# KenHBS/LDA_thesis

Measured on AMD Instinct MI355X. Metric: million tokens resampled/sec (Gibbs sweep), higher is better.
Workload: dtype f64-exact (fp32 tier 0 + fp64 tiers: the drawn topic is the fp64 pipeline's)

## Files before the change

### lda_thesis_amd/csrc/build_info.hpp

```cpp
#pragma once
#ifdef LLDA_MARGIN0
#define LLDA_INFO_MARGIN0 LLDA_BUILD_MARGIN0
#else
#define LLDA_INFO_MARGIN0 0
#endif
#ifdef LLDA_WAVES
#define LLDA_INFO_WAVES LLDA_BUILD_WAVES
#else
#define LLDA_INFO_WAVES 0
#endif
#ifdef LLDA_MARGIN0_WIDE
#define LLDA_INFO_MARGIN0_WIDE LLDA_BUILD_MARGIN0_WIDE
#else
#define LLDA_INFO_MARGIN0_WIDE 0
#endif
#ifdef ABL_NOLOAD
#define LLDA_INFO_NOLOAD LLDA_BUILD_ABL_NOLOAD
#else
#define LLDA_INFO_NOLOAD 0
#endif
#ifdef ABL_NOCOMMIT
#define LLDA_INFO_NOCOMMIT LLDA_BUILD_ABL_NOCOMMIT
#else
#define LLDA_INFO_NOCOMMIT 0
#endif
#ifdef ABL_WIDE_NOROW
#define LLDA_INFO_WIDE_NOROW LLDA_BUILD_ABL_WIDE_NOROW
#else
#define LLDA_INFO_WIDE_NOROW 0
#endif
#ifdef ABL_WIDE_NOADDLOAD
#define LLDA_INFO_WIDE_NOADDLOAD LLDA_BUILD_ABL_WIDE_NOADDLOAD
#else
#define LLDA_INFO_WIDE_NOADDLOAD 0
#endif
#ifdef ABL_NOFMA
#define LLDA_INFO_NOFMA LLDA_BUILD_ABL_NOFMA
#else
#define LLDA_INFO_NOFMA 0
#endif
#ifdef ABL_EXTRA_LDS_BYTES
#define LLDA_INFO_EXTRA_LDS LLDA_BUILD_ABL_EXTRA_LDS
#else
#define LLDA_INFO_EXTRA_LDS 0
#endif
#ifdef QUAD_PROFILE
#define LLDA_INFO_QUAD_PROFILE LLDA_BUILD_QUAD_PROFILE
#else
#define LLDA_INFO_QUAD_PROFILE 0
#endif
#ifdef LLDA_BUDGET_MARKS
#define LLDA_INFO_BUDGET_MARKS LLDA_BUILD_BUDGET_MARKS
#else
#define LLDA_INFO_BUDGET_MARKS 0
#endif
#ifdef LLDA_QUAD_PRIO
#define LLDA_INFO_QUAD_PRIO LLDA_BUILD_QUAD_PRIO
#else
#define LLDA_INFO_QUAD_PRIO 0
#endif
#define LLDA_BUILD_INFO_BITS (LLDA_INFO_QUAD_PRIO | LLDA_INFO_QUAD_PROFILE | LLDA_INFO_BUDGET_MARKS | LLDA_INFO_MARGIN0 | LLDA_INFO_WAVES | LLDA_INFO_MARGIN0_WIDE | LLDA_INFO_NOLOAD | LLDA_INFO_NOCOMMIT | \
                              LLDA_INFO_WIDE_NOROW | LLDA_INFO_WIDE_NOADDLOAD | LLDA_INFO_NOFMA | LLDA_INFO_EXTRA_LDS)
```

### lda_thesis_amd/csrc/kernel_quad.hpp

```cpp
#pragma once

namespace {

constexpr float LLDA_MARGIN0_QUAD = 0x1.ap-18f;
constexpr float QM_L = 1.05f * 32.0f * 0x1p-24f, QM_T = 1.05f * 39.0f * 0x1p-24f, QM_P = 1.05f * 37.0f * 0x1p-24f, QM_TOT = 1.05f * 0.25f * 0x1p-24f;
#define QLDS(arr, rho, t) (arr)[(rho) >> 2][t][(rho) & 3]
constexpr int QT = 32;
#ifdef LLDA_QUAD_PRIO
constexpr int QP_TOP = (LLDA_QUAD_PRIO) / 100 % 10, QP_DEC = (LLDA_QUAD_PRIO) / 10 % 10, QP_BULK = (LLDA_QUAD_PRIO) % 10;
#else
constexpr int QP_TOP = 3, QP_DEC = 0, QP_BULK = 2;
#endif
constexpr int QNT = 128;

template <int LB>
struct QuadGeo {
    static constexpr int LPD = 1 << LB;
    static constexpr int G = 2 * LPD;
    static constexpr int KP = 32 * LPD;
    static constexpr int IS = 3 + LB;
    static constexpr int DPW = 64 / LPD;
    static constexpr uint64_t GM = LPD == 64 ? ~0ull : ((1ull << LPD) - 1);
    static constexpr uint32_t KEY_NONE = 0xFC000u | 31u << 9 | (uint32_t)(KP - 1);
};

template <int LB>
__device__ __forceinline__ int quad_rho(int pos) { return ((pos >> LB) & 0x18) | ((pos & 3) << 1) | ((pos >> 2) & 1); }
constexpr int quad_rho_of(int i, int e, int c) { return 8 * i + 2 * c + e; }

template <int LB>
__device__ __forceinline__ uint32_t quad_min_key(uint32_t key)
{
    if constexpr (LB == 4)
        asm volatile("s_nop 1\n\tv_min_u32_dpp %0, %0, %0 row_ror:8 row_mask:0xf bank_mask:0xf\n\ts_nop 1\n\t"
                     "v_min_u32_dpp %0, %0, %0 row_ror:4 row_mask:0xf bank_mask:0xf\n\ts_nop 1\n\t"
                     "v_min_u32_dpp %0, %0, %0 row_ror:2 row_mask:0xf bank_mask:0xf\n\ts_nop 1\n\t"
                     "v_min_u32_dpp %0, %0, %0 row_ror:1 row_mask:0xf bank_mask:0xf" : "+v"(key));
    else if constexpr (LB == 3)
        asm volatile("s_nop 1\n\tv_min_u32_dpp %0, %0, %0 row_half_mirror row_mask:0xf bank_mask:0xf\n\ts_nop 1\n\t"
                     "v_min_u32_dpp %0, %0, %0 quad_perm:[1,0,3,2] row_mask:0xf bank_mask:0xf\n\ts_nop 1\n\t"
                     "v_min_u32_dpp %0, %0, %0 quad_perm:[2,3,0,1] row_mask:0xf bank_mask:0xf" : "+v"(key));
    else
        asm volatile("s_nop 1\n\tv_min_u32_dpp %0, %0, %0 quad_perm:[1,0,3,2] row_mask:0xf bank_mask:0xf\n\ts_nop 1\n\t"
                     "v_min_u32_dpp %0, %0, %0 quad_perm:[2,3,0,1] row_mask:0xf bank_mask:0xf" : "+v"(key));
    return key;
}

template <int LB>
struct QuadCounts {
    const int (*s_ndk)[QNT][4];
    const int *s_nk0;
    int t;
    int e;
    int g;
    bool st;
    __device__ __forceinline__ int word(int s) const { return QLDS(s_ndk, 8 * (s >> 2) + 2 * (s & 3) + e, t); }
    __device__ __forceinline__ int nd(int s) const { return word(s) & 0xffff; }
    __device__ __forceinline__ int nk(int s) const
    {
        const int w = word(s);
        return s_nk0[pos_of<QuadGeo<LB>::G, 16>(g, s)] + (w & 0xffff) - (int)((uint32_t)w >> 16);
    }
    __device__ __forceinline__ bool stats() const { return st; }
    __device__ __forceinline__ bool count_unsure() const { return false; }
};

template <int LB, bool PAD>
__device__ __noinline__ int quad_cold(const int (*s_ndk)[QNT][4], const int *s_nk0, int tbase, int w, int f, int zo, uint32_t ra,
                                      uint32_t rb, int lane, int64_t d, const KParams *P)
{
    constexpr int G = QuadGeo<LB>::G;
    const int g = lane & (G - 1);
    int x[16];
    gload_lane_row<G, 16>(P->n_kw, (int64_t)w * QuadGeo<LB>::KP, g, x);
    int lo, so;
    lane_slot_of<G, 16>(zo, lo, so);
#pragma unroll
    for (int s = 0; s < 16; ++s) x[s] -= (g == lo && s == so) ? f : 0;
    const QuadCounts<LB> dc{s_ndk, s_nk0, tbase + (g >> 1), g & 1, g, lane < G};
    if constexpr (PAD) return cold_tiers_acc<G, 16, true, false>(dc, x, P->lab_mask[d * G + g], uniform53(ra, rb), g, lane, P);
    else return cold_tiers_acc<G, 16, false, true>(dc, x, 0xFFFFu, uniform53(ra, rb), g, lane, P);
}

typedef float q_v2f __attribute__((ext_vector_type(2)));
typedef float q_v32f __attribute__((ext_vector_type(32)));

template <int LB, bool PAD = false>
__device__ __forceinline__ uint64_t quad_draw(const q_v32f &xv, const q_v2f (&pa)[16], float u, float margin_rel, float margin_data, float beta,
                                              int lq, int &zn)
{
    const q_v2f b2 = {beta, beta};
    q_v2f Q[16];
    LLDA_MARK("scores");
#pragma unroll
    for (int a = 0; a < 16; ++a) {
        const q_v2f x2 = {xv[2 * a], xv[2 * a + 1]};
        const q_v2f nb = x2 + b2;
        if (a == 0) Q[0] = nb * pa[0];
        else Q[a] = __builtin_elementwise_fma(nb, pa[a], Q[a - 1]);
    }
    LLDA_MARK("lane_scan");
    __builtin_amdgcn_s_setprio(QP_DEC);
    const float X0 = Q[15].x + Q[15].y;
    float X = X0;
    float tot = X0, prev;
    if constexpr (LB == 4) {
        X += dpp_f32<DPP_ROW_SHR + 1>(X);
        X += dpp_f32<DPP_ROW_SHR + 2>(X);
        X += dpp_f32<DPP_ROW_SHR + 4>(X);
        X += dpp_f32<DPP_ROW_SHR + 8>(X);
        tot += dpp_f32<DPP_ROW_ROR + 8>(tot);
        tot += dpp_f32<DPP_ROW_ROR + 4>(tot);
        tot += dpp_f32<DPP_ROW_ROR + 2>(tot);
        tot += dpp_f32<DPP_ROW_ROR + 1>(tot);
        prev = __int_as_float(__builtin_amdgcn_update_dpp(0, __float_as_int(X), DPP_ROW_SHR + 1, 0xF, 0xF, true));
    } else {
        const float m1 = lq >= 1 ? 1.0f : 0.0f, m2 = lq >= 2 ? 1.0f : 0.0f;
        X = __builtin_fmaf(dpp_f32<DPP_ROW_SHR + 1>(X), m1, X);
        X = __builtin_fmaf(dpp_f32<DPP_ROW_SHR + 2>(X), m2, X);
        if constexpr (LB == 3) {
            const float m4 = lq >= 4 ? 1.0f : 0.0f;
            X = __builtin_fmaf(dpp_f32<DPP_ROW_SHR + 4>(X), m4, X);
            tot += dpp_f32<DPP_HALF_MIRROR>(tot);
        }
        tot += dpp_f32<DPP_XOR1>(tot);
        tot += dpp_f32<DPP_XOR2>(tot);
        prev = dpp_f32<DPP_ROW_SHR + 1>(X) * m1;
    }
    LLDA_MARK("threshold");
    const float t = u * tot;
    const float tg = t - prev;
    const float md = __builtin_fmaf(QM_L, X0, __builtin_fmaf(QM_T, t, __builtin_fmaf(QM_P, prev, QM_TOT * tot)));
    const float margin = __builtin_fmaf(tot, margin_rel, margin_data * md);
    const float lo0 = tg - margin, hi0 = tg + margin;
    LLDA_MARK("search");
    const bool c0 = Q[15].x <= lo0;
    const float dA = c0 ? Q[15].x : 0.0f;
    const float lo = lo0 - dA, hi = hi0 - dA;
    float q[16];
#pragma unroll
    for (int a = 0; a < 16; ++a) q[a] = c0 ? Q[a].y : Q[a].x;
    const bool c5 = q[15] <= lo;
    float ub = c5 ? __int_as_float(0x7f800000) : q[15];
    const bool c1 = q[7] <= lo;
    ub = c1 ? ub : q[7];
    const float m2 = c1 ? q[11] : q[3];
    const float a1 = c1 ? q[9] : q[1], a5 = c1 ? q[13] : q[5];
    const float e0 = c1 ? q[8] : q[0], e2 = c1 ? q[10] : q[2], e4 = c1 ? q[12] : q[4], e6 = c1 ? q[14] : q[6];
    const bool c2 = m2 <= lo;
    ub = c2 ? ub : m2;
    const float m3 = c2 ? a5 : a1;
    const float g0 = c2 ? e4 : e0, g2 = c2 ? e6 : e2;
    const bool c3 = m3 <= lo;
    ub = c3 ? ub : m3;
    const float m4 = c3 ? g2 : g0;
    const bool c4 = m4 <= lo;
    ub = c4 ? ub : m4;
    uint64_t bad_total;
    asm("v_cmp_class_f32_e64 %0, %1, %2" : "=s"(bad_total) : "v"(tot - margin), "v"(0x2FF));
    uint64_t unsure = __ballot(!(ub > hi)) | bad_total;
    LLDA_MARK("pick");
    constexpr uint32_t I1 = 2u << QuadGeo<LB>::IS, I0 = 1u << QuadGeo<LB>::IS;
    const uint32_t p = (c1 ? (I1 | 16u << 9) : 0u) | (c2 ? (I0 | 8u << 9) : 0u) | (c3 ? (2u | 4u << 9) : 0u) | (c4 ? (1u | 2u << 9) : 0u) |
                       (c0 ? (4u | 1u << 9) : 0u) | ((uint32_t)lq << 3) | ((uint32_t)lq << 14);
    uint32_t key = c5 ? QuadGeo<LB>::KEY_NONE : p;
    key = quad_min_key<LB>(key);
    zn = (int)(key & 0x3FFFu);
    if constexpr (PAD) unsure |= __ballot(key == QuadGeo<LB>::KEY_NONE);
    return unsure;
}

template <int LB, bool PAD = false>
__device__ __forceinline__ uint64_t quad_tier1(const q_v32f &xv, const int (*s_ndk)[QNT][4], const int *s_nk0, int tid, int lq, double u,
                                               double alpha, double beta, double vbeta, double margin_rel, uint32_t vm, int &zn)
{
    double W[QT];
    double run = 0.0;
#pragma unroll
    for (int k = 0; k < QT; ++k) {
        const int e = k >> 4, a = k & 15, i = a >> 2, c = a & 3;
        const int rho = quad_rho_of(i, e, c);
        const int w = QLDS(s_ndk, rho, tid);
        const int nd = w & 0xffff, nk = s_nk0[(i << QuadGeo<LB>::IS) | (lq << 3) | (e << 2) | c] + nd - (int)((uint32_t)w >> 16);
        const double den = (double)nk + vbeta;
        double y = (double)__builtin_amdgcn_rcpf((float)den);
        y = __builtin_fma(__builtin_fma(-den, y, 1.0), y, y);
        y = __builtin_fma(__builtin_fma(-den, y, 1.0), y, y);
        const double ws = ((double)nd + alpha) * (((double)xv[rho] + beta) * y);
        run = run + (((vm >> k) & 1u) ? ws : 0.0);
        W[k] = run;
    }
    constexpr int LPD = QuadGeo<LB>::LPD;
    const double X = group_scan<LPD>(run, lq);
    const double tot = bcast_last<LPD>(X, tid & 63);
    double prev = dpp_f64<DPP_ROW_SHR + 1>(X);
    if constexpr (LB < 4) prev = lq ? prev : 0.0;
    const double tg = u * tot - prev;
    const double margin = tot * margin_rel;
    const double lo = tg - margin, hi = tg + margin;
    int cnt_lo = 0, cnt_hi = 0;
#pragma unroll
    for (int k = 0; k < QT; ++k) {
        cnt_lo += (W[k] <= lo) ? 1 : 0;
        cnt_hi += (W[k] <= hi) ? 1 : 0;
    }
    uint64_t unsure = __ballot((cnt_lo != cnt_hi) || !(tot > 0.0) || !(margin < tot));
    const uint32_t k = (uint32_t)cnt_lo;
    const uint32_t i_ = (k >> 2) & 3u, e_ = (k >> 4) & 1u, c_ = k & 3u;
    const uint32_t p = (i_ << QuadGeo<LB>::IS) | ((uint32_t)lq << 3) | (e_ << 2) | c_ | ((8u * i_ + 2u * c_ + e_) << 9) | ((uint32_t)lq << 14);
    uint32_t key = cnt_lo >= QT ? QuadGeo<LB>::KEY_NONE : p;
    key = quad_min_key<LB>(key);
    zn = (int)(key & 0x3FFFu);
    if constexpr (PAD) unsure |= __ballot(key == QuadGeo<LB>::KEY_NONE);
    return unsure;
}

struct QuadSite { int v, f, zo, c, zn, lo, so, w; };

#ifdef QUAD_PROFILE
#define QP_DECL uint32_t qp_t = 0, qp_acc[8] = {0, 0, 0, 0, 0, 0, 0, 0}
#define QP_START() do { __builtin_amdgcn_sched_barrier(0); qp_t = (uint32_t)__builtin_amdgcn_s_memtime(); __builtin_amdgcn_sched_barrier(0); } while (0)
#define QP_MARK(k) do { __builtin_amdgcn_sched_barrier(0); const uint32_t qp_n = (uint32_t)__builtin_amdgcn_s_memtime(); \
                        qp_acc[k] += qp_n - qp_t; qp_t = qp_n; __builtin_amdgcn_sched_barrier(0); } while (0)
#else
#define QP_DECL
#define QP_START()
#define QP_MARK(k)
#endif

template <int LB, bool REC = (LB < 4), bool PAD = false>
__global__ void __launch_bounds__(QNT, 2) llda_sweep_quad_kernel(const KParams P)
{
    typedef QuadGeo<LB> Geo;
    constexpr int KP = Geo::KP, LPD = Geo::LPD, G = Geo::G, IS = Geo::IS;
    __shared__ int s_nk[KP];
    __shared__ int s_nk0[KP];
    __shared__ int s_ndk[QT / 4][QNT][4];
    __shared__ float s_pa[QT / 4][QNT][4];
    __shared__ float s_u[QNT / LPD][2 * LPD];
    __shared__ int s_hot[QT][16];

    const int tid = threadIdx.x;
    for (int i = tid; i < KP; i += QNT) {
        s_nk[i] = 0;
        s_nk0[i] = P.n_k[i];
    }
    for (int i = tid; i < QT * 16; i += QNT) {
        const int so = i >> 4, k = i & 15;
        const int kk = ((so & 1) << 3) | ((so >> 4) << 2) | (((so >> 3) & 1) << 1) | ((so >> 2) & 1);
        s_hot[so][k] = k == kk ? -(1 << (((so >> 1) & 1) << 4)) : 0;
    }
    __syncthreads();

    const int lane = tid & 63, lq = tid & (LPD - 1), row = lane >> LB, grp = tid >> LB;
    const int gbase = lane & (64 - LPD);
    const float vbeta32 = (float)P.vbeta, alpha32 = (float)P.alpha, beta32 = (float)P.beta;

    const int64_t site_base = P.doc_off[0];
    const int32_t *word_b = P.word + site_base, *freq_b = P.freq + site_base, *csc_b = P.csc_pos + site_base;
    int32_t *z_b = P.z + site_base;

    typedef int v4i __attribute__((ext_vector_type(4)));
    QP_DECL;

    auto update = [&](int sg, int pos, int df) {
        const int w = QLDS(s_ndk, sg, tid) + df;
        QLDS(s_ndk, sg, tid) = w;
        const int nd = w & 0xffff, nk = s_nk0[pos] + nd - (int)((uint32_t)w >> 16);
        QLDS(s_pa, sg, tid) = tier0_factor(nd, nk, alpha32, vbeta32);
    };

    for (int it = 0; it < P.dpg; ++it) {
        const int64_t idx = ((int64_t)blockIdx.x * P.dpg + it) * (QNT / LPD) + grp;
        const bool valid = idx < P.D;
        const int64_t ic = valid ? idx : P.D - 1;
        const int64_t d = P.doc_order ? (int64_t)P.doc_order[ic] : ic;
        int64_t s0 = P.doc_off[d];
        int len = valid ? (int)(P.doc_off[d + 1] - s0) : 0;
        if (len <= 0) {
            len = 0;
            s0 = site_base;
        }
        int maxlen;
        if constexpr (LB == 4) {
            maxlen = max(max(__builtin_amdgcn_readlane(len, 0), __builtin_amdgcn_readlane(len, 16)),
                         max(__builtin_amdgcn_readlane(len, 32), __builtin_amdgcn_readlane(len, 48)));
        } else {
            int ml = len;
#pragma unroll
            for (int m = LPD; m < 64; m <<= 1) ml = max(ml, __shfl_xor(ml, m, 64));
            maxlen = __builtin_amdgcn_readfirstlane(ml);
        }
        if (maxlen == 0) continue;

        int32_t *ndk_row = P.n_dk + d * KP;
        const uint32_t vm = PAD ? (uint32_t)P.lab_mask[d * G + 2 * lq] | (uint32_t)P.lab_mask[d * G + 2 * lq + 1] << 16 : ~0u;
        {
            int big = 0, tokens = 0;
#pragma unroll
            for (int i = 0; i < 4; ++i) {
                const v4i a = ((const v4i *)ndk_row)[i * G + 2 * lq], b = ((const v4i *)ndk_row)[i * G + 2 * lq + 1];
                const int r[8] = {a.x, a.y, a.z, a.w, b.x, b.y, b.z, b.w};
#pragma unroll
                for (int j = 0; j < 8; ++j) {
                    const int rho = quad_rho_of(i, j >> 2, j & 3);
                    const int k = s_nk0[(i << IS) + lq * 8 + j];
                    QLDS(s_ndk, rho, tid) = r[j] | (r[j] << 16);
                    QLDS(s_pa, rho, tid) = ((vm >> (16 * (j >> 2) + 4 * i + (j & 3))) & 1u) ? tier0_factor(r[j], k, alpha32, vbeta32) : 0.0f;
                    big |= r[j];
                    tokens += (int)((uint32_t)r[j] & 0xffffu);
                }
            }
#pragma unroll
            for (int m = 1; m < LPD; m <<= 1) tokens += __shfl_xor(tokens, m, LPD);
            if (valid && (((uint32_t)big >> 16) || tokens > 65535) && P.status) atomicOr(P.status, 4);
        }
        const uint32_t gdoc = (uint32_t)(d + P.doc_base);
        const uint32_t sb = (uint32_t)(s0 - site_base) * 4u;
        const int last = len > 0 ? len - 1 : 0;
        auto off_of = [&](int n) { return opaque_u32(sb + (uint32_t)min(n, last) * 4u); };
        auto load_scalars = [&](QuadSite &R, const uint32_t o) {
            R.v = gload_i32(word_b, o); R.f = gload_i32(freq_b, o); R.c = gload_i32(csc_b, o); R.zo = gload_i32(z_b, o);
        };
        const int32_t *rec_b = REC ? P.site_rec + site_base * 4 : nullptr;
        int pv = 0, pf = 0, pc = 0;
        auto load_rec = [&](int &v, int &f, int &c, const uint32_t o) {
            const v4i r = *(const LLDA_GLOBAL v4i *)((const LLDA_GLOBAL char *)rec_b + (o << 2));
            v = r.x; f = r.y; c = r.z;
        };
        auto decode_old = [&](QuadSite &R) {
            R.lo = (R.zo >> 3) & (LPD - 1);
            R.so = quad_rho<LB>(R.zo);
        };
        int xp[16];
        auto load_row16 = [&](const int v, int &flag) {
#ifdef ABL_NOLOAD
#pragma unroll
            for (int k = 0; k < 16; ++k) xp[k] = ((v + k) & 7) * 0x10001;
            flag = 1;
            return;
#endif
            const LLDA_GLOBAL char *q = (const LLDA_GLOBAL char *)P.n_kw16 + (((uint32_t)v << (IS + 3)) + (uint32_t)lq * 16u);
            const v4i a = *(const LLDA_GLOBAL v4i *)q, b = *(const LLDA_GLOBAL v4i *)(q + 32 * LPD);
            const v4i c = *(const LLDA_GLOBAL v4i *)(q + 16 * LPD), e = *(const LLDA_GLOBAL v4i *)(q + 48 * LPD);
            xp[0] = a.x; xp[1] = a.y; xp[2] = a.z; xp[3] = a.w;
            xp[4] = b.x; xp[5] = b.y; xp[6] = b.z; xp[7] = b.w;
            xp[8] = c.x; xp[9] = c.y; xp[10] = c.z; xp[11] = c.w;
            xp[12] = e.x; xp[13] = e.y; xp[14] = e.z; xp[15] = e.w;
            flag = *(const LLDA_GLOBAL uint8_t *)((const LLDA_GLOBAL char *)P.row16 + (uint32_t)v);
        };
        q_v32f xv;
        auto convert_row = [&](const int v, const int flag, const int so, const float own) {
            LLDA_MARK("convert");
            const uint64_t wide_w = __ballot(flag == 0);
            if (__builtin_expect(wide_w == 0, 1)) {
#pragma unroll
                for (int k = 0; k < 16; ++k) {
                    const int e = k >> 3, j = (k >> 2) & 1, m = k & 3;
                    const int i = 2 * j + (m >> 1), c = 2 * (m & 1);
                    xv[quad_rho_of(i, e, c)] = (float)((uint32_t)xp[k] & 0xffffu);
                    xv[quad_rho_of(i, e, c + 1)] = (float)((uint32_t)xp[k] >> 16);
                }
            } else {
                LLDA_MARK("rare_wide_row");
                int xi[QT];
#pragma unroll
                for (int t = 0; t < QT; ++t) xi[t] = 0;
                if (flag == 0) {
                    const LLDA_GLOBAL v4i *q = (const LLDA_GLOBAL v4i *)((const LLDA_GLOBAL int32_t *)P.n_kw + ((uint64_t)(uint32_t)v << (IS + 2)));
#pragma unroll
                    for (int i = 0; i < 4; ++i) {
                        const v4i a = q[i * G + 2 * lq], b = q[i * G + 2 * lq + 1];
                        xi[quad_rho_of(i, 0, 0)] = a.x; xi[quad_rho_of(i, 0, 1)] = a.y; xi[quad_rho_of(i, 0, 2)] = a.z; xi[quad_rho_of(i, 0, 3)] = a.w;
                        xi[quad_rho_of(i, 1, 0)] = b.x; xi[quad_rho_of(i, 1, 1)] = b.y; xi[quad_rho_of(i, 1, 2)] = b.z; xi[quad_rho_of(i, 1, 3)] = b.w;
                    }
                }
#pragma unroll
                for (int k = 0; k < 16; ++k) {
                    const int e = k >> 3, j = (k >> 2) & 1, m = k & 3;
                    const int i = 2 * j + (m >> 1), c = 2 * (m & 1);
                    const int ra_ = quad_rho_of(i, e, c), rb_ = quad_rho_of(i, e, c + 1);
                    xv[ra_] = flag == 0 ? (float)xi[ra_] : (float)((uint32_t)xp[k] & 0xffffu);
                    xv[rb_] = flag == 0 ? (float)xi[rb_] : (float)((uint32_t)xp[k] >> 16);
                }
#pragma unroll
                for (int r = 0; r < QT; ++r) xv[r] -= (flag == 0 && so == r) ? own : 0.0f;
            }
        };
        auto remove_own_packed = [&](const int so, const int own) {
            LLDA_MARK("own_removal");
            const v4i *hot = (const v4i *)&s_hot[so][0];
#pragma unroll
            for (int j = 0; j < 4; ++j) {
                const v4i h = hot[j];
                xp[4 * j] += __mul24(h.x, own); xp[4 * j + 1] += __mul24(h.y, own);
                xp[4 * j + 2] += __mul24(h.z, own); xp[4 * j + 3] += __mul24(h.w, own);
            }
        };

        QuadSite R0, R1, R2;
        int wq = 0;
        if constexpr (REC) {
            load_rec(R0.v, R0.f, R0.c, off_of(0)); R0.zo = gload_i32(z_b, off_of(0));
            load_rec(R1.v, R1.f, R1.c, off_of(1)); R1.zo = gload_i32(z_b, off_of(1));
            load_rec(pv, pf, pc, off_of(2));
        } else {
            load_scalars(R0, off_of(0));
            load_scalars(R1, off_of(1));
            wq = gload_i32(word_b, off_of(2));
        }
        R0.zn = R1.zn = 0;
        R2.v = R2.f = R2.zo = R2.c = R2.zn = R2.lo = R2.so = R2.w = 0;
        load_row16(R0.v, R0.w);
        uint32_t r0 = 0, r1 = 0, r2 = 0, r3 = 0;
        decode_old(R0);
        if (len > 0 && lq == R0.lo) update(R0.so, R0.zo, -R0.f);
        remove_own_packed(R0.so, (len > 0 && lq == R0.lo) ? R0.f : 0);
        convert_row(R0.v, R0.w, R0.so, (len > 0 && lq == R0.lo) ? (float)R0.f : 0.0f);
        load_row16(R1.v, R1.w);

        auto site = [&](const int n, QuadSite &cur, QuadSite &nxt, QuadSite &prv) {
            const bool act = n < len, more = n + 1 < len;
            const int f = cur.f, zo = cur.zo;
            QP_START();
            LLDA_MARK("site_top");
            LLDA_MARK("lds_factors");
            __builtin_amdgcn_s_setprio(QP_TOP);
            q_v2f pa[16];
#pragma unroll
            for (int a = 0; a < 16; ++a) {
                pa[a].x = QLDS(s_pa, 2 * a, tid);
                pa[a].y = QLDS(s_pa, 2 * a + 1, tid);
            }
            LLDA_MARK("rng");
            if ((n & (2 * LPD - 1)) == 0) {
                LLDA_MARK("rare_philox");
                r0 = (uint32_t)(n >> 1) + (uint32_t)lq; r1 = gdoc; r2 = P.stream_id; r3 = P.sweep;
                philox4x32_10(r0, r1, r2, r3, P.key0, P.key1);
                s_u[grp][2 * lq] = (float)(r0 >> 5) * 0x1p-27f;
                s_u[grp][2 * lq + 1] = (float)(r2 >> 5) * 0x1p-27f;
                LLDA_MARK("rng");
            }
            const float u32 = s_u[grp][n & (2 * LPD - 1)];
            QP_MARK(0);
            int zn;
            uint64_t unsure = quad_draw<LB, PAD>(xv, pa, u32, P.margin0_rel, P.margin0_data, beta32, lq, zn) & __ballot(act);
            QP_MARK(1);
            LLDA_MARK("cold_check");
            if (__builtin_expect(unsure != 0, 0)) {
                LLDA_MARK("rare_cold");
                const int holder = (n >> 1) & (LPD - 1);
                const uint32_t ra_l = (n & 1) ? r2 : r0, rb_l = (n & 1) ? r3 : r1;
                const int bp_h = (gbase | holder) << 2;
                const uint32_t ra = (uint32_t)__builtin_amdgcn_ds_bpermute(bp_h, (int)ra_l), rb = (uint32_t)__builtin_amdgcn_ds_bpermute(bp_h, (int)rb_l);
                const uint64_t t0_w = unsure;
                if (lq == 0 && ((t0_w >> gbase) & Geo::GM) && P.status) atomicAdd(P.status + 1, 1);
                int z1;
                const uint64_t still = ((P.margin_rel < 1.0 ? quad_tier1<LB, PAD>(xv, s_ndk, s_nk0, tid, lq, uniform53(ra, rb), P.alpha, P.beta, P.vbeta,
                                                                        P.margin_rel, vm, z1) : ~0ull) | __ballot(cur.w == 0)) & __ballot(act);
                const bool mine0 = ((t0_w >> gbase) & Geo::GM) != 0;
                zn = mine0 ? z1 : zn;
                uint32_t rows = 0;
#pragma unroll
                for (int r = 0; r < Geo::DPW; ++r)
                    rows |= (((t0_w >> (LPD * r)) & Geo::GM) && ((still >> (LPD * r)) & Geo::GM)) ? (1u << r) : 0u;
                rows = (uint32_t)__builtin_amdgcn_readfirstlane((int)rows);
                while (__builtin_expect(rows != 0, 0)) {
                    const int r = __builtin_ctz(rows);
                    rows &= rows - 1;
                    const int src = r * LPD;
                    const int zo_r = __builtin_amdgcn_readlane(zo, src);
                    int zc = quad_cold<LB, PAD>(s_ndk, s_nk0, (tid & 64) + src, __builtin_amdgcn_readlane(cur.v, src),
                                       __builtin_amdgcn_readlane(f, src), zo_r, (uint32_t)__builtin_amdgcn_readlane((int)ra, src),
                                       (uint32_t)__builtin_amdgcn_readlane((int)rb, src), lane,
                                       (int64_t)__builtin_amdgcn_readlane((int)d, src),
                                       (const KParams *)__builtin_amdgcn_kernarg_segment_ptr());
                    if (__builtin_expect(zc < 0, 0)) {
                        zc = zo_r;
                        if (lane == 0 && P.status) atomicOr(P.status, 1);
                    }
                    zn = (row == r) ? (zc | (quad_rho<LB>(zc) << 9)) : zn;
                }
            }
            QP_MARK(2);
            LLDA_MARK("decode");

            {
                const int zpos = zn & 511, sn = zn >> 9, ln = (zn >> 3) & (LPD - 1);
                cur.zn = zpos;
                decode_old(nxt);
                const bool own_new = act && lq == ln, own_old = more && lq == nxt.lo;
                const int sg = own_new ? sn : own_old ? nxt.so : 0;
                const int ps = own_new ? zpos : own_old ? nxt.zo : (lq << 3);
                const int df = own_new ? f : own_old ? -nxt.f : 0;
                LLDA_MARK("count_update");
                const int w0 = QLDS(s_ndk, sg, tid), k0 = s_nk0[ps];
                QP_MARK(3);
                LLDA_MARK("scalars");
                __builtin_amdgcn_s_setprio(QP_BULK);
                int w_next;
                if constexpr (REC) {
                    prv.v = w_next = pv; prv.f = pf; prv.c = pc;
                    prv.zo = gload_i32(z_b, off_of(n + 2));
                    load_rec(pv, pf, pc, off_of(n + 3));
                } else {
                    w_next = wq;
                    load_scalars(prv, off_of(n + 2));
                    wq = gload_i32(word_b, off_of(n + 3));
                }
                QP_MARK(4);
                remove_own_packed(nxt.so, (more && lq == nxt.lo) ? nxt.f : 0);
                convert_row(nxt.v, nxt.w, nxt.so, (more && lq == nxt.lo) ? (float)nxt.f : 0.0f);
                QP_MARK(5);
                LLDA_MARK("row_prefetch");
                load_row16(w_next, prv.w);
                LLDA_MARK("count_update");
                const int w = w0 + df;
                QLDS(s_ndk, sg, tid) = w;
                const int nd = w & 0xffff, nk = k0 + nd - (int)((uint32_t)w >> 16);
                QLDS(s_pa, sg, tid) = tier0_factor(nd, nk, alpha32, vbeta32);
                if (__builtin_expect(__ballot(own_new && own_old) != 0, 0)) {
                    LLDA_MARK("rare_second_update");
                    if (own_new && own_old) update(nxt.so, nxt.zo, -nxt.f);
                }
#ifndef ABL_NOCOMMIT
                {
                    LLDA_MARK("commit");
                    const uint32_t zoff = opaque_u32(sb + (uint32_t)n * 4u);
                    const LLDA_GLOBAL uint32_t *lp = (const LLDA_GLOBAL uint32_t *)P.commit_log + (uint32_t)(cur.c & 0x7fffffff);
                    const uint32_t word = (uint32_t)zo | ((uint32_t)zpos << 16);
if (lq == 0 && act) {
                        gstore_i32(z_b, zoff, zpos);
                        *(LLDA_GLOBAL uint32_t *)lp = word;
                    }
                }
#endif
            }
            LLDA_MARK("loop");
            QP_MARK(6);
        };
        for (int n = 0;; n += 3) {
            site(n, R0, R1, R2);
            if (n + 1 >= maxlen) break;
            site(n + 1, R1, R2, R0);
            if (n + 2 >= maxlen) break;
            site(n + 2, R2, R0, R1);
            if (n + 3 >= maxlen) break;
        }

#ifdef QUAD_PROFILE
        if (blockIdx.x == 0 && tid == 0 && P.status) {
#pragma unroll
            for (int k = 0; k < 8; ++k) atomicAdd(P.status + 8 + k, (int)qp_acc[k]);
            atomicAdd(P.status + 16, maxlen);
        }
#endif
        if (valid && len > 0) {
#pragma unroll
            for (int i = 0; i < 4; ++i) {
                int o[8];
#pragma unroll
                for (int j = 0; j < 8; ++j) {
                    const int w = QLDS(s_ndk, quad_rho_of(i, j >> 2, j & 3), tid);
                    o[j] = w & 0xffff;
                    const int dl = o[j] - (int)((uint32_t)w >> 16);
                    if (dl) atomicAdd(&s_nk[(i << IS) + lq * 8 + j], dl);
                }
                v4i a = {o[0], o[1], o[2], o[3]}, b = {o[4], o[5], o[6], o[7]};
                ((v4i *)ndk_row)[i * G + 2 * lq] = a;
                ((v4i *)ndk_row)[i * G + 2 * lq + 1] = b;
            }
        }
    }

    __syncthreads();
    for (int i = tid; i < KP; i += QNT) {
        const int dl = s_nk[i];
        if (dl) atomicAdd(P.n_k_delta + i, dl);
    }
}

template <int G>
__global__ void __launch_bounds__(256) llda_pack_rows16_all_kernel(const int32_t *__restrict__ n_kw, uint16_t *__restrict__ out,
                                                                   uint8_t *__restrict__ row16, int64_t V)
{
    const int64_t t = (int64_t)blockIdx.x * 256 + threadIdx.x;
    const int64_t w = t / (2 * G);
    if (w >= V) return;
    const int c = (int)(t & (2 * G - 1)), j = c / G, g = c & (G - 1);
    const int4 *src = reinterpret_cast<const int4 *>(n_kw + w * (int64_t)(G * 16));
    const int4 a = src[(2 * j) * G + g], b = src[(2 * j + 1) * G + g];
    const int m = a.x | a.y | a.z | a.w | b.x | b.y | b.z | b.w;
    const uint64_t bal = __ballot((unsigned)m > 0xffffu);
    const int first = (int)(threadIdx.x & 63) & ~(2 * G - 1);
    const bool wide = G == 32 ? bal != 0 : ((bal >> first) & ((1ull << (2 * G % 64)) - 1)) != 0;
    uint4 o;
    o.x = ((uint32_t)a.x & 0xffffu) | ((uint32_t)a.y << 16);
    o.y = ((uint32_t)a.z & 0xffffu) | ((uint32_t)a.w << 16);
    o.z = ((uint32_t)b.x & 0xffffu) | ((uint32_t)b.y << 16);
    o.w = ((uint32_t)b.z & 0xffffu) | ((uint32_t)b.w << 16);
    reinterpret_cast<uint4 *>(out + w * (int64_t)(G * 16))[(2 * j + (g & 1)) * (G / 2) + (g >> 1)] = o;
    if (c == 0) row16[w] = wide ? 0 : 1;
}

}
```

### lda_thesis_amd/csrc/llda_gibbs.hip

```cpp
#include <hip/hip_runtime.h>
#include "build_info.hpp"
#ifndef ABL_EXTRA_LDS_BYTES
#define ABL_EXTRA_LDS_BYTES 0
#endif
#include <stdint.h>
#include <math.h>
#include <string.h>
#include <map>
#include <memory>
#include <type_traits>

#include "llda_gibbs.h"

#pragma clang fp contract(off)

#include "device_common.hpp"
#include "draw_tiers.hpp"
#include "exact_generic.hpp"
#include "kernel_sweep.hpp"
#include "kernel_quad.hpp"
#include "kernel_sparse.hpp"
#include "kernel_batch.hpp"
#include "kernel_readout.hpp"
#include "kernel_foldin.hpp"
// ... 492 lines not shown
                LLDA_WIDE_REG(2, true) LLDA_WIDE_REG(3, true) LLDA_WIDE_REG(4, true) LLDA_WIDE_REG(5, true)
                LLDA_WIDE_REG(6, true) LLDA_WIDE_REG(7, true) LLDA_WIDE_REG(8, true)
            default: return LLDA_E_BAD_K;
            }
        } else if (fast && a->debug_margin != -3) {
            switch (L.tiers) {
                LLDA_WIDE_REG(2, false) LLDA_WIDE_REG(3, false) LLDA_WIDE_REG(4, false) LLDA_WIDE_REG(5, false)
                LLDA_WIDE_REG(6, false) LLDA_WIDE_REG(7, false) LLDA_WIDE_REG(8, false)
            default: return LLDA_E_BAD_K;
            }
        } else if (fast) {
            rl = allow_lds(llda_sweep_wide_kernel<true>, lds);
            if (rl) return rl;
            hipLaunchKernelGGL(llda_sweep_wide_kernel<true>, grid, block, lds, st, W);
        } else {
            rl = allow_lds(llda_sweep_wide_kernel<false>, lds);
            if (rl) return rl;
            hipLaunchKernelGGL(llda_sweep_wide_kernel<false>, grid, block, lds, st, W);
        }
#undef LLDA_WIDE_REG
        const hipError_t e = hipGetLastError();
        return e == hipSuccess ? LLDA_OK : hip_fail(e);
    }

    const bool sparse = fast && !dense && a->live_off && a->live_pos && a->live_max >= 1 && a->live_max <= LLDA_MAX_LIVE;
    const int G = sparse ? (a->live_max <= 8 ? 8 : a->live_max <= 16 ? 16 : a->live_max <= 32 ? 32 : 64) : L.G;
    const int gpb = 256 / G;
    int dpg = a->docs_per_group;
    if (dpg < 1) dpg = 1;
    P.dpg = dpg;
    const int64_t per_block = (int64_t)gpb * dpg;
    const int64_t blocks = (a->D + per_block - 1) / per_block;
    if (blocks > 0x7fffffffLL) return LLDA_E_BAD_ARG;

    if (sparse) {
        P.live_off = a->live_off; P.live_pos = a->live_pos;
        if (a->debug_margin < 0) {
            P.margin_rel = 2.0;
            P.margin0_rel = 2.0f;
        }
        const dim3 grid((unsigned)blocks), block(256);
        const int rimg = take_image(a, P);
        if (rimg) return rimg;
#define LLDA_SPARSE(GS_)                                                                                              \
    case GS_:                                                                                                         \
        if (a->img_bits == 8) hipLaunchKernelGGL((llda_sweep_sparse_kernel<GS_, KParams, 8>), grid, block, 0, st, P);       \
        else if (a->img_bits == 16) hipLaunchKernelGGL((llda_sweep_sparse_kernel<GS_, KParams, 16>), grid, block, 0, st, P); \
        else hipLaunchKernelGGL((llda_sweep_sparse_kernel<GS_, KParams, 0>), grid, block, 0, st, P);                       \
        break;
        switch (G) { LLDA_SPARSE(8) LLDA_SPARSE(16) LLDA_SPARSE(32) LLDA_SPARSE(64) }
#undef LLDA_SPARSE
        const hipError_t e = hipGetLastError();
        return e == hipSuccess ? LLDA_OK : hip_fail(e);
    }
    if (a->n_kw_img || a->img_bits) return LLDA_E_BAD_ARG;
    if (a->row16) {
        if (!a->n_kw16 || a->site_row) return LLDA_E_BAD_ARG;
        if (!(fast && a->dense_mask != 0 && logged && llda_quad_ok(a->K))) return LLDA_E_BAD_ARG;
        if (a->D >= (1LL << 31)) return LLDA_E_BAD_ARG;
        P.quad_pad = L.K != L.KP;
        if (P.quad_pad && !P.lab_mask) return LLDA_E_BAD_ARG;
        if (!(a->max_doc_tokens > 0 && a->max_doc_tokens < 65536)) return LLDA_E_BAD_ARG;
        if ((reinterpret_cast<uintptr_t>(a->n_kw16) | reinterpret_cast<uintptr_t>(a->n_kw)) & 15) return LLDA_E_BAD_ARG;
        if (a->V >= (1LL << 22)) return LLDA_E_BAD_ARG;
        if (L.G <= 16 && !P.site_rec) return LLDA_E_BAD_ARG;
        if (a->n_sites < 1) return LLDA_OK;
        P.n_kw16 = a->n_kw16;
        P.row16 = a->row16;
        if (a->debug_margin == 0) {
            P.margin0_rel = 0.0f;
            P.margin0_data = 1.0f;
        } else if (a->debug_margin == -9) {
            P.margin0_rel = LLDA_MARGIN0_QUAD;
            P.margin_rel = 0x1p-40;
        } else if (a->debug_margin <= -10 && a->debug_margin >= -18) {
            P.margin0_rel = 0.0f;
            P.margin0_data = a->debug_margin == -10 ? 1.0f / 1.05f : ldexpf(1.0f, a->debug_margin + 10);
            P.margin_rel = 0x1p-40;
        }
        const int64_t per_q = (int64_t)(2 * QNT / L.G) * dpg;
        const int64_t qblocks = (a->D + per_q - 1) / per_q;
        if (qblocks > 0x7fffffffLL) return LLDA_E_BAD_ARG;
        const dim3 qgrid((unsigned)qblocks), qblock(QNT);
        if (!P.quad_pad) {
            if (L.G == 32) hipLaunchKernelGGL((llda_sweep_quad_kernel<4>), qgrid, qblock, 0, st, P);
            else if (L.G == 16) hipLaunchKernelGGL((llda_sweep_quad_kernel<3>), qgrid, qblock, 0, st, P);
            else hipLaunchKernelGGL((llda_sweep_quad_kernel<2>), qgrid, qblock, 0, st, P);
        } else {
            if (L.G == 32) hipLaunchKernelGGL((llda_sweep_quad_kernel<4, false, true>), qgrid, qblock, 0, st, P);
            else if (L.G == 16) hipLaunchKernelGGL((llda_sweep_quad_kernel<3, true, true>), qgrid, qblock, 0, st, P);
            else hipLaunchKernelGGL((llda_sweep_quad_kernel<2, true, true>), qgrid, qblock, 0, st, P);
        }
        const hipError_t e = hipGetLastError();
        return e == hipSuccess ? LLDA_OK : hip_fail(e);
    }
    if ((a->n_kw16 != nullptr) != (a->site_row != nullptr)) return LLDA_E_BAD_ARG;
    if (a->n_kw16) {
        if (!(fast && dense && logged && L.T == 16 && L.G >= 32)) return LLDA_E_BAD_ARG;
        if ((reinterpret_cast<uintptr_t>(a->n_kw16) | reinterpret_cast<uintptr_t>(a->n_kw)) & 15) return LLDA_E_BAD_ARG;
        P.n_kw16 = a->n_kw16;
        P.site_row = a->site_row;
        P.w4 = a->max_doc_tokens > 0 && a->max_doc_tokens < 65536 && a->debug_margin != -8;
    }
    switch (L.G) {
    case 8: return dispatch_sweep_T<8>(L.T, P, has_tail, fast, dense, blocks, st);
    case 16: return dispatch_sweep_T<16>(L.T, P, has_tail, fast, dense, blocks, st);
    case 32: return dispatch_sweep_T<32>(L.T, P, has_tail, fast, dense, blocks, st);
    case 64: return dispatch_sweep_T<64>(L.T, P, has_tail, fast, dense, blocks, st);
    }
    return LLDA_E_BAD_K;
}

int llda_sweep_batch(const llda_batch_args *a, void *stream)
{
    if (!a || a->n_inst < 0 || a->V < 1) return LLDA_E_BAD_ARG;
    if (a->n_inst == 0) return LLDA_OK;
    if (!a->inst_off || !a->order || !a->word || !a->freq || !a->z || !a->inst_prob || !a->inst_doc || !a->live_off ||
        !a->live_pos || !a->ndk_off || !a->n_dk || !a->kw_off || !a->nk_off || !a->kp || !a->prob_stream || !a->k || !a->counts ||
        !a->delta)
        return LLDA_E_BAD_ARG;
    if (a->lanes != 8 && a->lanes != 16 && a->lanes != 32 && a->lanes != 64) return LLDA_E_BAD_ARG;
    BParams P;
    memset(&P, 0, sizeof P);
    P.inst_off = a->inst_off; P.order = a->order; P.n_inst = a->n_inst; P.word = a->word; P.freq = a->freq; P.z = a->z;
    P.inst_prob = a->inst_prob; P.inst_doc = a->inst_doc; P.live_off = a->live_off; P.live_pos = a->live_pos;
    P.ndk_off = a->ndk_off; P.n_dk = a->n_dk; P.kw_off = a->kw_off; P.nk_off = a->nk_off; P.kp = a->kp;
    P.prob_stream = a->prob_stream; P.k = a->k;
    P.counts = a->counts; P.delta = a->delta; P.status = a->status;
    P.alpha = a->alpha; P.beta = a->beta; P.vbeta = (double)a->V * a->beta;
    if (!(a->alpha >= 1e-6 && a->beta >= 1e-6 && P.vbeta < 1099511627776.0)) return LLDA_E_BAD_ARG;
    P.margin_rel = a->debug_margin == 0 ? 0x1p-40 : (a->debug_margin > 0 ? ldexp(1.0, -a->debug_margin) : 2.0);
    P.key0 = (uint32_t)a->seed; P.key1 = (uint32_t)(a->seed >> 32); P.sweep = a->sweep;
    const int gpb = 256 / a->lanes;
    const int64_t blocks = (a->n_inst + gpb - 1) / gpb;
    if (blocks > 0x7fffffffLL) return LLDA_E_BAD_ARG;
    const dim3 grid((unsigned)blocks), block(256);
    hipStream_t st = (hipStream_t)stream;
    switch (a->lanes) {
    case 8: hipLaunchKernelGGL(llda_sweep_batch_kernel<8>, grid, block, 0, st, P); break;
    case 16: hipLaunchKernelGGL(llda_sweep_batch_kernel<16>, grid, block, 0, st, P); break;
    case 32: hipLaunchKernelGGL(llda_sweep_batch_kernel<32>, grid, block, 0, st, P); break;
    default: hipLaunchKernelGGL(llda_sweep_batch_kernel<64>, grid, block, 0, st, P); break;
    }
    const hipError_t e = hipGetLastError();
    return e == hipSuccess ? LLDA_OK : hip_fail(e);
}

int llda_commit_log(const int64_t *item_begin, const int32_t *item_len, const int32_t *item_word, int64_t n_items,
                    const uint32_t *commit_log, const int32_t *freq_csc, int32_t K, const int64_t *row_off,
                    int32_t *target, int32_t *n_k, int32_t *n_k_delta, void *stream)
{
    if (n_items < 0 || (n_k != nullptr) != (n_k_delta != nullptr)) return LLDA_E_BAD_ARG;
    int rc;
    const llda_layout *Lp = layout_of(K, &rc);
    if (rc) return rc;
    const llda_layout &L = *Lp;
    if (n_items > 0 && (!item_begin || !item_len || !item_word || !commit_log || !freq_csc || !target)) return LLDA_E_BAD_ARG;
    if (n_items == 0 && !n_k) return LLDA_OK;
    CParams P;
    P.item_begin = item_begin; P.item_len = item_len; P.item_word = item_word; P.n_items = n_items;
    P.log = commit_log; P.freq = freq_csc; P.row_off = row_off; P.target = target; P.n_k = n_k; P.n_k_delta = n_k_delta;
    P.KP = L.KP;
    int64_t blocks = (n_items + 3) / 4;
    if (blocks < 1) blocks = 1;
    if (blocks > 0x7fffffffLL) return LLDA_E_BAD_ARG;
    const int rl = allow_lds(llda_commit_log_kernel, 4 * L.KP * sizeof(int));
    if (rl) return rl;
    hipLaunchKernelGGL(llda_commit_log_kernel, dim3((unsigned)blocks), dim3(256), 4 * L.KP * sizeof(int), (hipStream_t)stream, P);
    const hipError_t e = hipGetLastError();
    return e == hipSuccess ? LLDA_OK : hip_fail(e);
}

int llda_apply_rows(const int64_t *row_off, int32_t *rows, int64_t n_rows, int32_t K, int32_t *counts, void *stream)
{
    if (n_rows < 0) return LLDA_E_BAD_ARG;
// ... 302 lines not shown
```

Measured before the change: 8930.

## Add unmasked full-length quad loop, compile out margin hooks, decode next site earlier

Adds a fast path in the quad sweep kernel. While every lane group still has at least five sites left, the loop runs an unmasked, unclamped variant that drops the act ballots and the min-clamped offsets. Debug margin hooks become a template parameter and are compiled out when debug_margin is zero. Old-topic decoding and z loads move one site earlier to shorten the dependency chain at each site. The cost is more code size and register pressure from the duplicated site instantiations and the extra template variants.

```diff
diff --git a/lda_thesis_amd/csrc/build_info.hpp b/lda_thesis_amd/csrc/build_info.hpp
--- a/lda_thesis_amd/csrc/build_info.hpp
+++ b/lda_thesis_amd/csrc/build_info.hpp
@@ -54,7 +54,7 @@
 #else
 #define LLDA_INFO_BUDGET_MARKS 0
 #endif
-#ifdef LLDA_QUAD_PRIO
+#if defined(LLDA_QUAD_PRIO) || defined(LLDA_QUAD_PARTS)
 #define LLDA_INFO_QUAD_PRIO LLDA_BUILD_QUAD_PRIO
 #else
 #define LLDA_INFO_QUAD_PRIO 0
diff --git a/lda_thesis_amd/csrc/kernel_quad.hpp b/lda_thesis_amd/csrc/kernel_quad.hpp
--- a/lda_thesis_amd/csrc/kernel_quad.hpp
+++ b/lda_thesis_amd/csrc/kernel_quad.hpp
@@ -12,6 +12,13 @@
 constexpr int QP_TOP = 3, QP_DEC = 0, QP_BULK = 2;
 #endif
 constexpr int QNT = 128;
+#ifdef LLDA_QUAD_PARTS
+constexpr int QUAD_PARTS = (LLDA_QUAD_PARTS);
+#else
+constexpr int QUAD_PARTS = 7;
+#endif
+constexpr bool QUAD_FULL_LOOP = (QUAD_PARTS & 1) != 0, QUAD_HOOKS_OUT = (QUAD_PARTS & 2) != 0, QUAD_EARLY_DECODE = (QUAD_PARTS & 4) != 0;
+template <bool B> struct QuadForm { static constexpr bool value = B; };
 
 template <int LB>
 struct QuadGeo {
@@ -85,7 +92,7 @@
 typedef float q_v2f __attribute__((ext_vector_type(2)));
 typedef float q_v32f __attribute__((ext_vector_type(32)));
 
-template <int LB, bool PAD = false>
+template <int LB, bool PAD = false, bool HOOKS = true>
 __device__ __forceinline__ uint64_t quad_draw(const q_v32f &xv, const q_v2f (&pa)[16], float u, float margin_rel, float margin_data, float beta,
                                               int lq, int &zn)
 {
@@ -131,7 +138,8 @@
     const float t = u * tot;
     const float tg = t - prev;
     const float md = __builtin_fmaf(QM_L, X0, __builtin_fmaf(QM_T, t, __builtin_fmaf(QM_P, prev, QM_TOT * tot)));
-    const float margin = __builtin_fmaf(tot, margin_rel, margin_data * md);
+    float margin = md;
+    if constexpr (HOOKS) margin = __builtin_fmaf(tot, margin_rel, margin_data * md);
     const float lo0 = tg - margin, hi0 = tg + margin;
     LLDA_MARK("search");
     const bool c0 = Q[15].x <= lo0;
@@ -215,7 +223,7 @@
     return unsure;
 }
 
-struct QuadSite { int v, f, zo, c, zn, lo, so, w; };
+struct QuadSite { int v, f, zo, c, zn, lo, so; uint8_t w; };
 
 #ifdef QUAD_PROFILE
 #define QP_DECL uint32_t qp_t = 0, qp_acc[8] = {0, 0, 0, 0, 0, 0, 0, 0}
@@ -228,7 +236,7 @@
 #define QP_MARK(k)
 #endif
 
-template <int LB, bool REC = (LB < 4), bool PAD = false>
+template <int LB, bool REC = (LB < 4), bool PAD = false, bool HOOKS = false>
 __global__ void __launch_bounds__(QNT, 2) llda_sweep_quad_kernel(const KParams P)
 {
     typedef QuadGeo<LB> Geo;
@@ -238,7 +246,9 @@
     __shared__ int s_ndk[QT / 4][QNT][4];
     __shared__ float s_pa[QT / 4][QNT][4];
     __shared__ float s_u[QNT / LPD][2 * LPD];
-    __shared__ int s_hot[QT][16];
+    __shared__ __attribute__((aligned(16))) int s_hot[QT][16];
+    static_assert(LB != 4 || sizeof(s_nk) + sizeof(s_nk0) + sizeof(s_ndk) + sizeof(s_pa) + sizeof(s_u) + sizeof(s_hot) <= 40960,
+                  "K = 512: the static LDS of a workgroup must leave room for four workgroups on a CU");
 
     const int tid = threadIdx.x;
     for (int i = tid; i < KP; i += QNT) {
@@ -281,15 +291,21 @@
             len = 0;
             s0 = site_base;
         }
-        int maxlen;
+        int maxlen, minlen;
         if constexpr (LB == 4) {
-            maxlen = max(max(__builtin_amdgcn_readlane(len, 0), __builtin_amdgcn_readlane(len, 16)),
-                         max(__builtin_amdgcn_readlane(len, 32), __builtin_amdgcn_readlane(len, 48)));
+            const int l0 = __builtin_amdgcn_readlane(len, 0), l1 = __builtin_amdgcn_readlane(len, 16);
+            const int l2 = __builtin_amdgcn_readlane(len, 32), l3 = __builtin_amdgcn_readlane(len, 48);
+            maxlen = max(max(l0, l1), max(l2, l3));
+            minlen = min(min(l0, l1), min(l2, l3));
         } else {
-            int ml = len;
-#pragma unroll
-            for (int m = LPD; m < 64; m <<= 1) ml = max(ml, __shfl_xor(ml, m, 64));
+            int ml = len, nl = len;
+#pragma unroll
+            for (int m = LPD; m < 64; m <<= 1) {
+                ml = max(ml, __shfl_xor(ml, m, 64));
+                nl = min(nl, __shfl_xor(nl, m, 64));
+            }
             maxlen = __builtin_amdgcn_readfirstlane(ml);
+            minlen = __builtin_amdgcn_readfirstlane(nl);
         }
         if (maxlen == 0) continue;
 
@@ -319,6 +335,7 @@
         const uint32_t sb = (uint32_t)(s0 - site_base) * 4u;
         const int last = len > 0 ? len - 1 : 0;
         auto off_of = [&](int n) { return opaque_u32(sb + (uint32_t)min(n, last) * 4u); };
+        auto off_full = [&](int n) { return opaque_u32(sb + (uint32_t)n * 4u); };
         auto load_scalars = [&](QuadSite &R, const uint32_t o) {
             R.v = gload_i32(word_b, o); R.f = gload_i32(freq_b, o); R.c = gload_i32(csc_b, o); R.zo = gload_i32(z_b, o);
         };
@@ -333,7 +350,7 @@
             R.so = quad_rho<LB>(R.zo);
         };
         int xp[16];
-        auto load_row16 = [&](const int v, int &flag) {
+        auto load_row16 = [&](const int v, uint8_t &flag) {
 #ifdef ABL_NOLOAD
 #pragma unroll
             for (int k = 0; k < 16; ++k) xp[k] = ((v + k) & 7) * 0x10001;
@@ -350,7 +367,7 @@
             flag = *(const LLDA_GLOBAL uint8_t *)((const LLDA_GLOBAL char *)P.row16 + (uint32_t)v);
         };
         q_v32f xv;
-        auto convert_row = [&](const int v, const int flag, const int so, const float own) {
+        auto convert_row = [&](const int v, const uint8_t flag, const int so, const float own) {
             LLDA_MARK("convert");
             const uint64_t wide_w = __ballot(flag == 0);
             if (__builtin_expect(wide_w == 0, 1)) {
@@ -411,19 +428,30 @@
         }
         R0.zn = R1.zn = 0;
         R2.v = R2.f = R2.zo = R2.c = R2.zn = R2.lo = R2.so = R2.w = 0;
+        if constexpr (QUAD_EARLY_DECODE) {
+            R2.v = REC ? pv : wq;
+            R2.zo = gload_i32(z_b, off_of(2));
+        }
         load_row16(R0.v, R0.w);
         uint32_t r0 = 0, r1 = 0, r2 = 0, r3 = 0;
         decode_old(R0);
+        if constexpr (QUAD_EARLY_DECODE) decode_old(R1);
         if (len > 0 && lq == R0.lo) update(R0.so, R0.zo, -R0.f);
         remove_own_packed(R0.so, (len > 0 && lq == R0.lo) ? R0.f : 0);
         convert_row(R0.v, R0.w, R0.so, (len > 0 && lq == R0.lo) ? (float)R0.f : 0.0f);
         load_row16(R1.v, R1.w);
 
-        auto site = [&](const int n, QuadSite &cur, QuadSite &nxt, QuadSite &prv) {
-            const bool act = n < len, more = n + 1 < len;
+        auto site = [&](auto form, const int n, QuadSite &cur, QuadSite &nxt, QuadSite &prv) {
+            constexpr bool FULL = decltype(form)::value;
+            const bool act = FULL || n < len, more = FULL || n + 1 < len;
+            auto off = [&](int m) { if constexpr (FULL) return off_full(m); else return off_of(m); };
             const int f = cur.f, zo = cur.zo;
             QP_START();
-            LLDA_MARK("site_top");
+            if constexpr (FULL || !QUAD_FULL_LOOP) {
+                LLDA_MARK("site_top");
+            } else {
+                LLDA_MARK("site_top_masked");
+            }
             LLDA_MARK("lds_factors");
             __builtin_amdgcn_s_setprio(QP_TOP);
             q_v2f pa[16];
@@ -444,7 +472,10 @@
             const float u32 = s_u[grp][n & (2 * LPD - 1)];
             QP_MARK(0);
             int zn;
-            uint64_t unsure = quad_draw<LB, PAD>(xv, pa, u32, P.margin0_rel, P.margin0_data, beta32, lq, zn) & __ballot(act);
+            uint64_t unsure;
+            if constexpr (HOOKS) unsure = quad_draw<LB, PAD, true>(xv, pa, u32, P.margin0_rel, P.margin0_data, beta32, lq, zn);
+            else unsure = quad_draw<LB, PAD, false>(xv, pa, u32, 0.0f, 1.0f, beta32, lq, zn);
+            if constexpr (!FULL) unsure &= __ballot(act);
             QP_MARK(1);
             LLDA_MARK("cold_check");
             if (__builtin_expect(unsure != 0, 0)) {
@@ -456,8 +487,9 @@
                 const uint64_t t0_w = unsure;
                 if (lq == 0 && ((t0_w >> gbase) & Geo::GM) && P.status) atomicAdd(P.status + 1, 1);
                 int z1;
-                const uint64_t still = ((P.margin_rel < 1.0 ? quad_tier1<LB, PAD>(xv, s_ndk, s_nk0, tid, lq, uniform53(ra, rb), P.alpha, P.beta, P.vbeta,
-                                                                        P.margin_rel, vm, z1) : ~0ull) | __ballot(cur.w == 0)) & __ballot(act);
+                uint64_t still = ((!HOOKS || P.margin_rel < 1.0 ? quad_tier1<LB, PAD>(xv, s_ndk, s_nk0, tid, lq, uniform53(ra, rb), P.alpha, P.beta, P.vbeta,
+                                                                                  P.margin_rel, vm, z1) : ~0ull) | __ballot(cur.w == 0));
+                if constexpr (!FULL) still &= __ballot(act);
                 const bool mine0 = ((t0_w >> gbase) & Geo::GM) != 0;
                 zn = mine0 ? z1 : zn;
                 uint32_t rows = 0;
@@ -488,7 +520,9 @@
             {
                 const int zpos = zn & 511, sn = zn >> 9, ln = (zn >> 3) & (LPD - 1);
                 cur.zn = zpos;
-                decode_old(nxt);
+                uint32_t cword = (uint32_t)zo | ((uint32_t)zpos << 16);
+                asm volatile("" : "+v"(cword));
+                if constexpr (!QUAD_EARLY_DECODE) decode_old(nxt);
                 const bool own_new = act && lq == ln, own_old = more && lq == nxt.lo;
                 const int sg = own_new ? sn : own_old ? nxt.so : 0;
                 const int ps = own_new ? zpos : own_old ? nxt.zo : (lq << 3);
@@ -501,13 +535,19 @@
                 int w_next;
                 if constexpr (REC) {
                     prv.v = w_next = pv; prv.f = pf; prv.c = pc;
-                    prv.zo = gload_i32(z_b, off_of(n + 2));
-                    load_rec(pv, pf, pc, off_of(n + 3));
+                    if constexpr (QUAD_EARLY_DECODE) cur.zo = gload_i32(z_b, off(n + 3));
+                    else prv.zo = gload_i32(z_b, off(n + 2));
+                    load_rec(pv, pf, pc, off(n + 3));
+                } else if constexpr (QUAD_EARLY_DECODE) {
+                    w_next = prv.v;
+                    prv.f = gload_i32(freq_b, off(n + 2)); prv.c = gload_i32(csc_b, off(n + 2));
+                    cur.v = gload_i32(word_b, off(n + 3)); cur.zo = gload_i32(z_b, off(n + 3));
                 } else {
                     w_next = wq;
-                    load_scalars(prv, off_of(n + 2));
-                    wq = gload_i32(word_b, off_of(n + 3));
-                }
+                    load_scalars(prv, off(n + 2));
+                    wq = gload_i32(word_b, off(n + 3));
+                }
+                if constexpr (QUAD_EARLY_DECODE) decode_old(prv);
                 QP_MARK(4);
                 remove_own_packed(nxt.so, (more && lq == nxt.lo) ? nxt.f : 0);
                 convert_row(nxt.v, nxt.w, nxt.so, (more && lq == nxt.lo) ? (float)nxt.f : 0.0f);
@@ -528,8 +568,8 @@
                     LLDA_MARK("commit");
                     const uint32_t zoff = opaque_u32(sb + (uint32_t)n * 4u);
                     const LLDA_GLOBAL uint32_t *lp = (const LLDA_GLOBAL uint32_t *)P.commit_log + (uint32_t)(cur.c & 0x7fffffff);
-                    const uint32_t word = (uint32_t)zo | ((uint32_t)zpos << 16);
-if (lq == 0 && act) {
+                    const uint32_t word = cword;
+                    if (lq == 0 && act) {
                         gstore_i32(z_b, zoff, zpos);
                         *(LLDA_GLOBAL uint32_t *)lp = word;
                     }
@@ -539,12 +579,20 @@
             LLDA_MARK("loop");
             QP_MARK(6);
         };
-        for (int n = 0;; n += 3) {
-            site(n, R0, R1, R2);
+        int n = 0;
+        if constexpr (QUAD_FULL_LOOP) {
+            for (; n + 5 < minlen; n += 3) {
+                site(QuadForm<true>{}, n, R0, R1, R2);
+                site(QuadForm<true>{}, n + 1, R1, R2, R0);
+                site(QuadForm<true>{}, n + 2, R2, R0, R1);
+            }
+        }
+        for (;; n += 3) {
+            site(QuadForm<false>{}, n, R0, R1, R2);
             if (n + 1 >= maxlen) break;
-            site(n + 1, R1, R2, R0);
+            site(QuadForm<false>{}, n + 1, R1, R2, R0);
             if (n + 2 >= maxlen) break;
-            site(n + 2, R2, R0, R1);
+            site(QuadForm<false>{}, n + 2, R2, R0, R1);
             if (n + 3 >= maxlen) break;
         }
 
diff --git a/lda_thesis_amd/csrc/llda_gibbs.hip b/lda_thesis_amd/csrc/llda_gibbs.hip
--- a/lda_thesis_amd/csrc/llda_gibbs.hip
+++ b/lda_thesis_amd/csrc/llda_gibbs.hip
@@ -598,15 +598,22 @@
         const int64_t qblocks = (a->D + per_q - 1) / per_q;
         if (qblocks > 0x7fffffffLL) return LLDA_E_BAD_ARG;
         const dim3 qgrid((unsigned)qblocks), qblock(QNT);
+        const bool hooks = a->debug_margin != 0 || !QUAD_HOOKS_OUT;
+#define LLDA_QUAD(LB_, REC_, PAD_)                                                                                                    \
+        do {                                                                                                                           \
+            if (hooks) hipLaunchKernelGGL((llda_sweep_quad_kernel<LB_, REC_, PAD_, true>), qgrid, qblock, 0, st, P);                   \
+            else hipLaunchKernelGGL((llda_sweep_quad_kernel<LB_, REC_, PAD_, false>), qgrid, qblock, 0, st, P);                        \
+        } while (0)
         if (!P.quad_pad) {
-            if (L.G == 32) hipLaunchKernelGGL((llda_sweep_quad_kernel<4>), qgrid, qblock, 0, st, P);
-            else if (L.G == 16) hipLaunchKernelGGL((llda_sweep_quad_kernel<3>), qgrid, qblock, 0, st, P);
-            else hipLaunchKernelGGL((llda_sweep_quad_kernel<2>), qgrid, qblock, 0, st, P);
+            if (L.G == 32) LLDA_QUAD(4, false, false);
+            else if (L.G == 16) LLDA_QUAD(3, true, false);
+            else LLDA_QUAD(2, true, false);
         } else {
-            if (L.G == 32) hipLaunchKernelGGL((llda_sweep_quad_kernel<4, false, true>), qgrid, qblock, 0, st, P);
-            else if (L.G == 16) hipLaunchKernelGGL((llda_sweep_quad_kernel<3, true, true>), qgrid, qblock, 0, st, P);
-            else hipLaunchKernelGGL((llda_sweep_quad_kernel<2, true, true>), qgrid, qblock, 0, st, P);
-        }
+            if (L.G == 32) LLDA_QUAD(4, false, true);
+            else if (L.G == 16) LLDA_QUAD(3, true, true);
+            else LLDA_QUAD(2, true, true);
+        }
+#undef LLDA_QUAD
         const hipError_t e = hipGetLastError();
         return e == hipSuccess ? LLDA_OK : hip_fail(e);
     }
```

After: 9269 (median of 6 runs). +3.8%, better.
